# maleiwhat/Our-Tree

Measured on AMD Instinct MI355X. Metric: GB/s AES-128-CTR (whole node), higher is better.
Workload: dtype uint8

## Files before the change

csrc/cpu/bs_selftest.cpp:

```cpp
#include <stdio.h>
#include <stdlib.h>
#include <string.h>

#include "aes.h"
#include "otc_bitslice.h"

using namespace otc_bs;

extern "C" int otc_bitslice_selftest(int verbose)
{
    const uint8_t *SB = aes_sbox();
    int fails = 0;
    for (int batch = 0; batch < 8; ++batch) {
        W x[8] = {0};
        for (int k = 0; k < 32; ++k) {
            int v = batch * 32 + k;
            for (int i = 0; i < 8; ++i) x[i] |= (W)((v >> i) & 1) << k;
        }
        sbox(x[0], x[1], x[2], x[3], x[4], x[5], x[6], x[7]);
        for (int k = 0; k < 32; ++k) {
            int v = batch * 32 + k, o = 0;
            for (int i = 0; i < 8; ++i) o |= (int)((x[i] >> k) & 1) << i;
            if (o != SB[v]) {
                if (verbose) printf("  sbox mismatch at %02x: %02x vs %02x\n", v, o, SB[v]);
                ++fails;
            }
        }
    }
    for (int kv = 0; kv < 256; kv += 37) {
        W k[8], x[8] = {0}, y[8];
        for (int i = 0; i < 8; ++i) k[i] = ((kv >> i) & 1) ? ~0u : 0u;
        for (int slot = 0; slot < 32; ++slot)
            for (int i = 0; i < 8; ++i) x[i] |= (W)(((slot * 7 + kv) >> i) & 1) << slot;
        for (int i = 0; i < 8; ++i) y[i] = x[i] ^ k[i];
        sbox(y[0], y[1], y[2], y[3], y[4], y[5], y[6], y[7]);
        W z[8];
        for (int i = 0; i < 8; ++i) z[i] = x[i];
        sbox_k<false>(x[0], x[1], x[2], x[3], x[4], x[5], x[6], x[7], k[0], k[1], k[2], k[3], k[4], k[5], k[6], k[7]);
        sbox_lut3(z[0], z[1], z[2], z[3], z[4], z[5], z[6], z[7], k[0], k[1], k[2], k[3], k[4], k[5], k[6], k[7]);
        for (int i = 0; i < 8; ++i)
            if (x[i] != y[i] || z[i] != y[i]) {
                if (verbose) printf("  sbox_k/sbox_lut3 mismatch kv=%d bit %d\n", kv, i);
                ++fails;
            }
    }
    for (int t = 0; t < 64; ++t) {
        W a[32], b[32];
        uint64_t z = 0x9E3779B97F4A7C15ull * (uint64_t)(t + 1);
        for (int i = 0; i < 32; ++i) {
            z ^= z << 13; z ^= z >> 7; z ^= z << 17;
            a[i] = b[i] = (W)(z >> 11);
        }
        transpose32(a);
        transpose32_ref(b);
        for (int i = 0; i < 32; ++i)
            if (a[i] != b[i]) {
                if (verbose) printf("  transpose32 mismatch (trial %d, word %d)\n", t, i);
                ++fails;
                break;
            }
    }
    srand(7);
    for (int bits = 128; bits <= 256; bits += 64) {
        unsigned char key[32], pt[32][16], ref[32][16];
        for (int i = 0; i < 32; ++i) key[i] = (unsigned char)rand();
        for (int k = 0; k < 32; ++k)
            for (int i = 0; i < 16; ++i) pt[k][i] = (unsigned char)rand();
        aes_context ctx;
        aes_setkey_enc(&ctx, key, (unsigned)bits);
        for (int k = 0; k < 32; ++k) aes_crypt_ecb(&ctx, AES_ENCRYPT, pt[k], ref[k]);
        uint32_t rk[60];
        aes_export_rk32(&ctx, rk);
        W s[128];
        for (int w = 0; w < 4; ++w) {
            W m[32];
            for (int k = 0; k < 32; ++k) memcpy(&m[k], &pt[k][4 * w], 4);
            transpose32(m);
            for (int q = 0; q < 32; ++q) s[32 * w + q] = m[q];
        }
        W km[128];
        key_masks(rk, km);
        for (int p = 0; p < 128; ++p) s[p] ^= km[p];
        for (int r = 1; r < ctx.nr; ++r) {
            key_masks(rk + 4 * r, km);
            round_full(s, km);
        }
        key_masks(rk + 4 * ctx.nr, km);
        round_last(s, km);
        int bad = 0;
        for (int w = 0; w < 4; ++w) {
            W m[32];
            for (int q = 0; q < 32; ++q) m[q] = s[32 * w + q];
            transpose32(m);
            for (int k = 0; k < 32; ++k) bad += memcmp(&m[k], &ref[k][4 * w], 4) != 0;
        }
        if (verbose) printf("  bitsliced AES-%d (32 blocks): %s\n", bits, bad ? "failed" : "passed");
        fails += bad;

        for (int w = 0; w < 4; ++w) {
            W m[32];
            for (int k = 0; k < 32; ++k) memcpy(&m[k], &pt[k][4 * w], 4);
            transpose32(m);
            for (int q = 0; q < 32; ++q) s[32 * w + q] = m[q];
        }
        auto kf = [&](int r, int p) -> W { return (W)(0u - ((rk[4 * r + (p >> 5)] >> (p & 31)) & 1u)); };
        if (ctx.nr == 10) encrypt_planes<10, false>(s, kf);
        else if (ctx.nr == 12) encrypt_planes<12, false>(s, kf);
        else encrypt_planes<14, false>(s, kf);
        bad = 0;
        for (int w = 0; w < 4; ++w) {
            W m[32];
            for (int q = 0; q < 32; ++q) m[q] = s[32 * w + q];
            transpose32(m);
            for (int k = 0; k < 32; ++k) {
                uint32_t v = m[k] ^ rk[4 * ctx.nr + w];
                bad += memcmp(&v, &ref[k][4 * w], 4) != 0;
            }
        }
        if (verbose) printf("  bitsliced AES-%d kernel schedule: %s\n", bits, bad ? "failed" : "passed");
        fails += bad;

        for (int mixt = 0; mixt < 3; ++mixt) {
            for (int w = 0; w < 4; ++w) {
                W m[32];
                for (int k = 0; k < 32; ++k) memcpy(&m[k], &pt[k][4 * w], 4);
                transpose32(m);
                for (int q = 0; q < 32; ++q) s[32 * w + q] = m[q];
            }
            for (int r = 0; r + 1 < ctx.nr; ++r) {
                auto kr = [&](int p) -> W { return kf(r, p); };
                if (mixt == 2) round_step<2>(s, kr);
                else if (mixt == 1) round_step<1>(s, kr);
                else round_step<0>(s, kr);
            }
            round_final(s, [&](int p) -> W { return kf(ctx.nr - 1, p); });
            bad = 0;
            for (int w = 0; w < 4; ++w) {
                W m[32];
                for (int q = 0; q < 32; ++q) m[q] = s[32 * w + q];
                transpose32(m);
// ... 102 lines not shown
```

csrc/hip/aes_bs.hip:

```cpp
#include <hip/hip_runtime.h>

#include <cstdlib>
#include <cstring>
#include <type_traits>

#include "otc_bitslice.h"
#include "otc_device.h"
#include "otc_kernels.h"

using namespace otc_dev;
using namespace otc_bs;

namespace {

struct BsParams {
    const uint8_t *in;
    uint8_t *out;
    uint64_t nblocks;
    uint32_t tail;
    uint32_t wrap64;
    uint64_t shift;
    Ctr128 cbase;
    const uint32_t *ktab;
    const uint32_t *ctab;
// ... 149 lines not shown
    __device__ __forceinline__ void operator()(int b, W *t) const
    {
        ktab_ptr q = tp;
        asm volatile("" : "+s"(q));
#pragma unroll
        for (int j = 0; j < OTC_SBOX_KEY_TERMS; ++j) t[j] = q[(R * 16 + b) * OTC_BS_KT_STRIDE + j];
    }
};

template <int BASE>
struct GroupTerms {
    ktab_ptr gp;
    __device__ __forceinline__ void operator()(int b, W *t) const
    {
        ktab_ptr q = gp;
        asm volatile("" : "+s"(q));
#pragma unroll
        for (int j = 0; j < OTC_SBOX_KEY_TERMS; ++j) t[j] = q[(BASE + b) * OTC_BS_KT_STRIDE + j];
    }
};

__global__ __launch_bounds__(256) void k_bs_ctr_table(otc_aes_key K, Ctr128 cbase, uint32_t wrap64,
                                                      uint64_t ngroups, uint64_t tasks, uint32_t *gtab,
                                                      uint32_t *e0tab, uint32_t *e1tab)
{
    __shared__ uint32_t sbt[256];
    sbt[threadIdx.x] = sbox_value(threadIdx.x);
    __syncthreads();
    const auto sb = [&](uint32_t v) { return sbt[v & 0xFFu]; };
    const uint64_t i = (uint64_t)blockIdx.x * 256u + threadIdx.x;
    auto rk0b = [&](int b) -> uint32_t { return (K.rk[b >> 2] >> (8 * (b & 3))) & 0xFFu; };
    uint64_t g;
    int kind;
    if (i < ngroups) {
        g = i;
        kind = 0;
    } else if (i < ngroups * 65) {
        g = (i - ngroups) >> 6;
        kind = 1;
    } else if (i < ngroups * 65 + tasks) {
        g = (((cbase.lo >> 11) & 31u) + (i - ngroups * 65)) >> 5;
        kind = 2;
    } else {
        return;
    }
    uint8_t pre[14];
    ctr_group_prefix(cbase.lo, cbase.hi, wrap64 != 0, g, pre);
    uint32_t c8[8];
    if (kind == 0) {
        ctr_group_consts(pre, K.rk, sb, c8, gtab + g * OTC_BS_CTR_GRP_WORDS);
    } else if (kind == 1) {
        ctr_group_consts(pre, K.rk, sb, c8, (uint32_t *)nullptr);
        const uint32_t lane = (uint32_t)(i - ngroups) & 63u;
        ctr_e0_lane(c8, rk0b(15), lane, sb, e0tab + (g * 64 + lane) * 8);
    } else {
        ctr_group_consts(pre, K.rk, sb, c8, (uint32_t *)nullptr);
        const uint64_t t = i - ngroups * 65;
        const uint32_t u5 = (uint32_t)((cbase.lo >> 11) + t) & 31u;
        ctr_e1_task(c8, rk0b(14), u5, sb, e1tab + t * OTC_BS_CTR_E1_WORDS);
    }
}

template <int R, int NR, int MIX, bool DEC = false>
__device__ __forceinline__ void rounds_table(W *s, ktab_ptr tp)
{
    if constexpr (R < NR - 1) {
        round_step_kt<MIX, TableTerms<R>, 2, DEC>(s, TableTerms<R>{tp});
        pin_n(s, 128);
        rounds_table<R + 1, NR, MIX, DEC>(s, tp);
    } else {
        round_final_kt<TableTerms<NR - 1>, DEC>(s, TableTerms<NR - 1>{tp});
    }
}

#ifndef OTC_BS_CBC_D
#define OTC_BS_CBC_D 4
#endif
#ifndef OTC_BS_CFB_D
#define OTC_BS_CFB_D 2
#endif
#ifndef OTC_BS_PRE
#define OTC_BS_PRE 2
#endif
template <int NR, int MODE, int LS, bool CACHE, bool FO, int MIX = 2, int PRE = OTC_BS_PRE, int D = 8>
__device__ __forceinline__ void aes_bs_task(const BsParams &P, const otc_aes_key &K, uint4 *stage,
                                            int64_t claimed = -1)
{
    Task t;
    if (!task_of<MODE>(P, t, claimed)) return;
    const uint32_t lane = t.lane, wave = t.wave;
    const uint64_t shift = (MODE == BS_CTR) ? P.shift : 0;
    const bool full = FO || t.full;
    W s[128];
    auto prefetch = [&]() {
    if (MODE == BS_CTR && LS > 0) {
        const int64_t t0 = (int64_t)t.vbase - (int64_t)shift;
        const uint8_t *ib0 = P.in + t0 * 16 + lane * 16u;
#pragma unroll
        for (int k = 0; k < LS; ++k) {
            const int64_t si = t0 + (int64_t)lane + 64 * k;
            const bool ok = full || (si >= 0 && (uint64_t)si < P.nblocks);
            __builtin_amdgcn_global_load_lds((const void *)(ok ? ib0 + 1024u * k : P.in),
                                             (__attribute__((address_space(3))) void *)&stage[(wave * LS + k) * 64],
                                             16, 0, BS_LDS_AUX);
        }
    }
    };
    if (!(MODE == BS_CTR && CACHE)) prefetch();
    if (MODE == BS_CTR && CACHE) {
        const uint64_t task = t.vbase >> 11;
        const uint64_t g = (((P.cbase.lo >> 11) & 31u) + task) >> 5;
        const uint4 *q0 = (const uint4 *)(P.e0tab + (g * 64u + lane) * 8u);
        const uint4 a = q0[0], b = q0[1];
        const W ew[8] = {a.x, a.y, a.z, a.w, b.x, b.y, b.z, b.w};
        W e0[32];
#pragma unroll
        for (int p = 0; p < 32; ++p) e0[p] = rep_byte(ew[p >> 2], p & 3);
        const ktab_ptr e1p = (ktab_ptr)P.e1tab + task * OTC_BS_CTR_E1_WORDS;
        W e1[32];
#pragma unroll
        for (int p = 0; p < 32; ++p) e1[p] = e1p[p];
        const ktab_ptr gp = (ktab_ptr)P.ctab + g * OTC_BS_CTR_GRP_WORDS;
        ctr_round2_mix(e0, e1, s);
        pin_n(s, 128);
        sched_fence();
        prefetch();
        sched_fence();
        round_step_kt<MIX, GroupTerms<0>, 2>(s, GroupTerms<0>{gp});
        pin_n(s, 128);
        sched_fence();
        rounds_table<3, NR, MIX>(s, (ktab_ptr)P.ktab);
    } else if (MODE == BS_CTR) {
        const uint64_t clo = P.cbase.lo + t.vbase;
        const uint64_t chi = P.cbase.hi + ((!P.wrap64 && clo < P.cbase.lo) ? 1u : 0u);
        uint32_t cw[4] = {(uint32_t)clo, (uint32_t)(clo >> 32), (uint32_t)chi, (uint32_t)(chi >> 32)};
#pragma unroll
        for (int j = 0; j < 4; ++j) asm volatile("" : "+v"(cw[j]));
#pragma unroll
        for (int b = 0; b < 16; ++b) {
#pragma unroll
            for (int i = 0; i < 8; ++i) {
                const int n = 8 * (15 - b) + i;
                W v;
                if (n < 6) {
                    v = lane_mask(lane, n);
                } else if (n < 11) {
                    constexpr W pat[5] = {0xAAAAAAAAu, 0xCCCCCCCCu, 0xF0F0F0F0u, 0xFF00FF00u, 0xFFFF0000u};
                    v = pat[n - 6];
                } else {
                    v = (W)(0u - ((cw[n >> 5] >> (n & 31)) & 1u));
                }
                s[8 * b + i] = v;
            }
        }
#pragma unroll
        for (int q = 0; q < 128; ++q) asm volatile("" : "+v"(s[q]));
    } else {
        ecb_load_planes<MODE>(P, t, s, full);
    }
    constexpr bool DEC = MODE == BS_ECB_DEC || is_cbcd<MODE>;
    if (DEC) {
        dec_premap(s);
        pin_n(s, 128);
    }
    if (!(MODE == BS_CTR && CACHE)) {
        sched_fence();
        rounds_table<0, NR, MIX, DEC>(s, (ktab_ptr)P.ktab);
    }
    pin_n(s, 128);
    sched_fence();

    const int64_t tstart = (int64_t)t.vbase - (int64_t)shift;
    const uint8_t *ib = P.in + tstart * 16;
    uint8_t *ob = P.out + tstart * 16;
    uint32_t lo = lane * 16u;
    asm volatile("" : "+v"(lo));
    auto slot_ok = [&](int k) {
        const int64_t si = tstart + (int64_t)lane + 64 * k;
        return full || (si >= 0 && (uint64_t)si < P.nblocks);
    };
    constexpr bool XIN = MODE == BS_CTR || is_cbcd<MODE> || is_cfbd<MODE>;
    constexpr int XOFF = MODE == BS_CBC_DEC ? -16 : 0;
    uint4 pt[32];
    auto issue = [&](int j) {
        if (XIN && j >= LS && j < 32) {
            if constexpr (MODE == BS_CBC_DEC_SEG) {
                pt[j] = seg_prev<MODE>(P, ib + lo + 1024u * j, (uint64_t)(tstart + lane + 64 * j),
                                       slot_ok(j));
            } else if (MODE == BS_CBC_DEC && j == 0) {
                const bool first = tstart + lane == 0;
                const uint4 v = slot_ok(j) ? *(const uint4 *)(ib + lo + (first ? 0 : XOFF)) : make_uint4(0, 0, 0, 0);
                pt[j] = blend_iv(v, first, P);
            } else {
                pt[j] = slot_ok(j) ? ld_stream(ib + lo + 1024u * j + XOFF) : make_uint4(0, 0, 0, 0);
            }
        }
    };
    constexpr bool REG_XIN = is_cbcd<MODE> || is_cfbd<MODE>;
    constexpr int PRE_ = REG_XIN ? 0 : PRE, D_ = is_cfbd<MODE> ? OTC_BS_CFB_D : REG_XIN ? OTC_BS_CBC_D : D;
#pragma unroll
    for (int j = 0; j < LS + PRE_; ++j) issue(j);
    sched_fence();
#pragma unroll
    for (int w = 0; w < 4; ++w) {
        transpose32(s + 32 * w);
        pin_n(s + 32 * w, 32);
        sched_fence();
    }
    constexpr uint32_t KD = DEC ? 0x05050505u : 0u;
    const uint32_t k0 = K.rk[4 * NR + 0] ^ KD, k1 = K.rk[4 * NR + 1] ^ KD, k2 = K.rk[4 * NR + 2] ^ KD,
                   k3 = K.rk[4 * NR + 3] ^ KD;
    auto ks_xor = [&](int k, uint4 x) {
        uint4 o;
        o.x = x3(x.x, s[k], k0);
        o.y = x3(x.y, s[32 + k], k1);
        o.z = x3(x.z, s[64 + k], k2);
        o.w = x3(x.w, s[96 + k], k3);
        return o;
    };
#pragma unroll
    for (int k = 0; k < 32; ++k) {
        if ((k & 3) == 0) {
            sched_fence();
#pragma unroll
            for (int j = LS + PRE_; j < 32; ++j)
                if ((j - D_ < 0 ? 0 : ((j - D_) & ~3)) == k) issue(j);
        }
        if (slot_ok(k)) {
            const uint4 o = XIN ? ks_xor(k, k < LS ? stage[(wave * LS + k) * 64 + (lo >> 4)] : pt[k])
                                : make_uint4(s[k] ^ k0, s[32 + k] ^ k1, s[64 + k] ^ k2, s[96 + k] ^ k3);
            st_stream(ob + lo + 1024u * k, o);
        }
    }
}

#ifndef OTC_BS_LS
#define OTC_BS_LS 8
#endif
constexpr int BS_LS = OTC_BS_LS;


template <int NR, int MODE, int LS, bool CACHE, bool FO>
__global__ __launch_bounds__(256) __attribute__((amdgpu_waves_per_eu(3, 3))) void k_aes_bs_t3(BsParams P,
                                                                                             otc_aes_key K)
{
    __shared__ uint4 stage[LS > 0 ? BS_WPG * LS * 64 : 1];
    aes_bs_task<NR, MODE, LS, CACHE, FO>(P, K, stage);
}

template <int NR, int MODE>
__global__ __launch_bounds__(256) __attribute__((amdgpu_waves_per_eu(3, 3))) void k_aes_bs_claim(BsParams P,
                                                                                               otc_aes_key K)
{
    strace(3);
    const uint32_t w = blockIdx.x * 4u + __builtin_amdgcn_readfirstlane(threadIdx.x >> 6);
    for (int64_t u = first_unit(P.cl, false, w); u >= 0; u = claim_unit(P.cl, false)) {
        BsParams Q = P;
        auto gin = (__attribute__((address_space(1))) const uint8_t *)P.in;
        auto gout = (__attribute__((address_space(1))) uint8_t *)P.out;
        asm volatile("" : "+s"(gin), "+s"(gout));
        Q.in = (const uint8_t *)gin;
        Q.out = (uint8_t *)gout;
        aes_bs_task<NR, MODE, 0, false, true>(Q, K, nullptr, u);
    }
}

template <int NR, int MODE>
hipError_t launch_nr(const BsParams &P, const otc_aes_key &K, hipStream_t st)
{
    const uint64_t vt = P.nblocks + (MODE == BS_CTR ? P.shift : 0);
    const uint64_t tasks = (vt + 2047) / 2048;
    uint64_t wgs = (tasks + BS_WPG - 1) / BS_WPG;
    if (wgs < 1) wgs = 1;
    if (wgs > 0xFFFFFFFFull) return hipErrorInvalidValue;
    const dim3 g((unsigned)wgs), b(64 * BS_WPG);
    bool cache = MODE == BS_CTR;
    const uint64_t ngroups = cache ? (((P.cbase.lo >> 11) & 31u) + tasks + 31) >> 5 : 0;
    const size_t ctab_words =
        cache ? ngroups * (OTC_BS_CTR_GRP_WORDS + OTC_BS_CTR_E0_WORDS) + tasks * OTC_BS_CTR_E1_WORDS : 0;
    const size_t kt_words = (size_t)NR * 16 * OTC_BS_KT_STRIDE;
    uint32_t *tab = nullptr;
    hipError_t e = hipErrorOutOfMemory;
    if (cache) {
        e = alloc_fault() ? hipErrorOutOfMemory : hipMallocAsync((void **)&tab, (kt_words + ctab_words) * 4, st);
        if (e != hipSuccess) {
            (void)hipGetLastError();
            cache = false;
        }
    }
    if (!cache) e = alloc_fault() ? hipErrorOutOfMemory : hipMallocAsync((void **)&tab, kt_words * 4, st);
    if (e != hipSuccess) return e;
    hipLaunchKernelGGL(k_bs_key_table<MODE == BS_ECB_DEC || is_cbcd<MODE>>, dim3(1), dim3(256), 0, st, K, tab);
    BsParams Q = P;
    Q.ktab = tab;
    Q.tasks = tasks;
    constexpr int LS = MODE == BS_CTR ? BS_LS : 0;
    if constexpr (MODE != BS_CTR) {
        (void)g;
        if (!P.cl.ctr) {
            (void)hipFreeAsync(tab, st);
            return hipErrorInvalidValue;
        }
        hipLaunchKernelGGL((k_aes_bs_claim<NR, MODE>),
                           dim3(P.cl.wgs ? P.cl.wgs : (unsigned)otc_dev::device_cus()), dim3(256), 0, st, Q, K);
    } else {
        const bool edge = P.shift != 0 || vt % 2048 != 0;
        auto run = [&](auto cachec) {
            constexpr bool C = decltype(cachec)::value;
            Q.part = BS_FULL_ONLY;
            hipLaunchKernelGGL((k_aes_bs_t3<NR, MODE, LS, C, true>), g, b, 0, st, Q, K);
            if (edge) {
                Q.part = BS_EDGE_ONLY;
                hipLaunchKernelGGL((k_aes_bs_t3<NR, MODE, LS, C, false>), dim3((2 + BS_WPG - 1) / BS_WPG), b, 0, st,
                                   Q, K);
// ... 93 lines not shown
```

csrc/include/otc.h:

```cpp
#ifndef OTC_H
#define OTC_H

#include <stddef.h>
#include <stdint.h>

#ifdef __cplusplus
extern "C" {
#endif

#define OTC_OK 0
#define OTC_ERR_ARG -1
#define OTC_ERR_HIP -2
#define OTC_ERR_RCCL -3
#define OTC_ERR_UNSUPPORTED -4
#define OTC_ERR_NOMEM -5

const char *otc_last_error(void);

#define OTC_DIR_ENCRYPT 1
#define OTC_DIR_DECRYPT 0

typedef struct {
    uint32_t rk[60];
    int32_t nr;
// ... 156 lines not shown
int otc_device_clock_khz(int dev);
int otc_set_device(int dev);
int otc_device_sync(void);
void *otc_stream_create(void);
void otc_stream_destroy(void *stream);
int otc_stream_join(void *a, void *b);

typedef struct otc_engine otc_engine;

otc_engine *otc_engine_create(int device, size_t chunk_bytes, int depth);
#define OTC_ENGINE_DEFAULT 0
#define OTC_ENGINE_POOLED_QUEUES 1
otc_engine *otc_engine_create_ex(int device, size_t chunk_bytes, int depth, int flags);
void otc_engine_destroy(otc_engine *e);

#define OTC_MODE_ECB 0
#define OTC_MODE_CTR 1
#define OTC_MODE_CBC_DEC 2
#define OTC_MODE_XOR 3

typedef struct {
    double total_ms;
    double kernel_ms;
    double h2d_ms, d2h_ms;
    double host_stage_ms;
    size_t bytes;
    int chunks;
    int numa_node;
} otc_stream_stats;

int otc_engine_run(otc_engine *e, int mode, const void *host_in, void *host_out, size_t nbytes,
                   const otc_aes_key *k, const uint8_t iv_or_ctr[16], uint64_t block_offset,
                   int impl, otc_stream_stats *stats);

int otc_device_numa_node(int dev);
int otc_engine_numa_node(const otc_engine *e);
const void *otc_engine_staging(const otc_engine *e, int slot);

#define OTC_PTR_HOST 0
#define OTC_PTR_PINNED 1
#define OTC_PTR_DEVICE 2
int otc_ptr_kind(const void *p);

int otc_host_register(void *p, size_t nbytes);
int otc_host_unregister(void *p);
void *otc_host_alloc_pinned(size_t nbytes);
void otc_host_free_pinned(void *p);

typedef struct {
    double total_ms;
    double gbps;
    int ngpus;
    int strategy;
    int numa_nodes_used;
} otc_multi_stats;

int otc_multi_run(int ngpus, int strategy, int mode, const void *host_in, void *host_out,
                  size_t nbytes, const otc_aes_key *k, const uint8_t iv_or_ctr[16], int impl,
                  size_t chunk_bytes, otc_multi_stats *stats);

typedef struct {
    uint64_t round_off;
    uint64_t round_bytes;
    uint64_t pad_bytes;
    uint64_t off, bytes;
    uint64_t blk0;
    int64_t halo;
} otc_rccl_piece;
uint64_t otc_rccl_nrounds(uint64_t nbytes, int ngpus, uint64_t piece);
int otc_rccl_plan_piece(uint64_t nbytes, int ngpus, uint64_t piece, uint64_t r, int g, otc_rccl_piece *out);
uint64_t otc_rccl_halo_start(uint64_t nbytes, uint64_t piece, uint64_t i);

void otc_multi_release(void);
void otc_release_resources(void);

void otc_fault_inject_alloc(long after);
long otc_fault_inject_pending(void);

int otc_multi_ctr_resident(int ngpus, void *const *dev_bufs, size_t shard_bytes,
                           const otc_aes_key *k, const uint8_t ctr0[16], int impl,
                           double *elapsed_ms);

int otc_bitslice_selftest(int verbose);
const char *otc_build_info(void);
int otc_runtime_info(char *buf, size_t n);

#ifdef __cplusplus
}
#endif

#endif
```

csrc/include/otc_bitslice.h:

```cpp
#ifndef OTC_BITSLICE_H
#define OTC_BITSLICE_H

#include <stdint.h>

#if defined(__HIPCC__) || defined(__HIP__)
#define OTC_HD __host__ __device__ __forceinline__
#else
#define OTC_HD inline
#endif



namespace otc_bs {

typedef uint32_t W;

OTC_HD void sbox(W &x0, W &x1, W &x2, W &x3, W &x4, W &x5, W &x6, W &x7)
{
    const W U0 = x7, U1 = x6, U2 = x5, U3 = x4, U4 = x3, U5 = x2, U6 = x1, U7 = x0;
    const W T1 = U0 ^ U3, T2 = U0 ^ U5, T3 = U0 ^ U6, T4 = U3 ^ U5, T5 = U4 ^ U6;
    const W T6 = T1 ^ T5, T7 = U1 ^ U2, T8 = U7 ^ T6, T9 = U7 ^ T7, T10 = T6 ^ T7;
    const W T11 = U1 ^ U5, T12 = U2 ^ U5, T13 = T3 ^ T4, T14 = T6 ^ T11, T15 = T5 ^ T11;
    const W T16 = T5 ^ T12, T17 = T9 ^ T16, T18 = U3 ^ U7, T19 = T7 ^ T18, T20 = T1 ^ T19;
    const W T21 = U6 ^ U7, T22 = T7 ^ T21, T23 = T2 ^ T22, T24 = T2 ^ T10, T25 = T20 ^ T17;
// ... 578 lines not shown
}

OTC_HD void key_masks(const uint32_t *rk4, W *k)
{
#pragma unroll
    for (int b = 0; b < 16; ++b) {
        uint32_t byte = (rk4[b >> 2] >> (8 * (b & 3))) & 0xffu;
#pragma unroll
        for (int i = 0; i < 8; ++i) k[8 * b + i] = ((byte >> i) & 1u) ? ~0u : 0u;
    }
}

struct ArrayKey {
    const W *k;
    OTC_HD W operator()(int p) const { return k[p]; }
};

OTC_HD void round_full(W *s, const W *k)
{
    W t[128];
    sub_bytes(s);
    shift_rows(s, t);
    mix_columns_ark(t, s, ArrayKey{k});
}

OTC_HD void round_last(W *s, const W *k)
{
    W t[128];
    sub_bytes(s);
    shift_rows(s, t);
#pragma unroll
    for (int p = 0; p < 128; ++p) s[p] = t[p] ^ k[p];
}

OTC_HD W perm_b(W hi, W lo, uint32_t sel)
{
#if defined(__HIP_DEVICE_COMPILE__)
    return __builtin_amdgcn_perm(hi, lo, sel);
#else
    W r = 0;
    for (int i = 0; i < 4; ++i) {
        const uint32_t s = (sel >> (8 * i)) & 0xFFu;
        const W byte = s < 4 ? (lo >> (8 * s)) & 0xFFu : (hi >> (8 * (s - 4))) & 0xFFu;
        r |= byte << (8 * i);
    }
    return r;
#endif
}

OTC_HD W bsel(W m, W x, W y) { return (x & m) | (y & ~m); }

template <int J>
OTC_HD void transpose_bits(W *m, W mk)
{
#pragma unroll
    for (int k = 0; k < 32; ++k) {
        if (k & J) continue;
        const W a = m[k], b = m[k | J];
        m[k] = bsel(mk << J, b << J, a);
        m[k | J] = bsel(mk, a >> J, b);
    }
}

OTC_HD void transpose32(W *m)
{
#pragma unroll
    for (int k = 0; k < 16; ++k) {
        const W a = m[k], b = m[k | 16];
        m[k] = perm_b(b, a, 0x05040100u);
        m[k | 16] = perm_b(b, a, 0x07060302u);
    }
#pragma unroll
    for (int k = 0; k < 32; ++k) {
        if (k & 8) continue;
        const W a = m[k], b = m[k | 8];
        m[k] = perm_b(b, a, 0x06020400u);
        m[k | 8] = perm_b(b, a, 0x07030501u);
    }
    transpose_bits<4>(m, 0x0F0F0F0Fu);
    transpose_bits<2>(m, 0x33333333u);
    transpose_bits<1>(m, 0x55555555u);
}

inline void transpose32_ref(W *m)
{
    W t[32] = {0};
    for (int r = 0; r < 32; ++r)
        for (int c = 0; c < 32; ++c) t[c] |= ((m[r] >> c) & 1u) << r;
    for (int i = 0; i < 32; ++i) m[i] = t[i];
}

}

#endif
```

our_tree_amd/_native.py:

```python
from __future__ import annotations

import atexit
import ctypes
import os
import threading

_HERE = os.path.dirname(os.path.abspath(__file__))
LIB_DIR = os.path.join(_HERE, "lib")
GPU_LIB_PATH = os.environ.get("OTC_LIB") or os.path.join(LIB_DIR, "libotc.so")
CPU_LIB_PATH = os.path.join(LIB_DIR, "libotc_cpu.so")

_lock = threading.Lock()
_gpu_lib = None
_cpu_lib = None

c_u8p = ctypes.POINTER(ctypes.c_uint8)
c_vp = ctypes.c_void_p
c_sz = ctypes.c_size_t
c_u64 = ctypes.c_uint64
c_int = ctypes.c_int


class OtcAesKey(ctypes.Structure):

# ... 49 lines not shown

    _fields_ = [("nonce_counter", ctypes.c_uint8 * 16), ("stream_block", ctypes.c_uint8 * 16),
                ("nc_off", ctypes.c_size_t)]


class StreamStats(ctypes.Structure):
    _fields_ = [
        ("total_ms", ctypes.c_double),
        ("kernel_ms", ctypes.c_double),
        ("h2d_ms", ctypes.c_double),
        ("d2h_ms", ctypes.c_double),
        ("host_stage_ms", ctypes.c_double),
        ("bytes", ctypes.c_size_t),
        ("chunks", ctypes.c_int),
        ("numa_node", ctypes.c_int),
    ]


class RcclPiece(ctypes.Structure):
    _fields_ = [
        ("round_off", ctypes.c_uint64),
        ("round_bytes", ctypes.c_uint64),
        ("pad_bytes", ctypes.c_uint64),
        ("off", ctypes.c_uint64),
        ("bytes", ctypes.c_uint64),
        ("blk0", ctypes.c_uint64),
        ("halo", ctypes.c_int64),
    ]


class MultiStats(ctypes.Structure):
    _fields_ = [
        ("total_ms", ctypes.c_double),
        ("gbps", ctypes.c_double),
        ("ngpus", ctypes.c_int),
        ("strategy", ctypes.c_int),
        ("numa_nodes_used", ctypes.c_int),
    ]


def _declare_cpu(lib):
    P = ctypes.POINTER
    sig = {
        "aes_setkey_enc": (c_int, [P(AesContext), c_u8p, ctypes.c_uint]),
        "aes_setkey_dec": (c_int, [P(AesContext), c_u8p, ctypes.c_uint]),
        "aes_crypt_ecb": (c_int, [P(AesContext), c_int, c_u8p, c_u8p]),
        "aes_crypt_cbc": (c_int, [P(AesContext), c_int, c_sz, c_u8p, c_u8p, c_u8p]),
        "aes_crypt_cfb128": (c_int, [P(AesContext), c_int, c_sz, P(c_int), c_u8p, c_u8p, c_u8p]),
        "aes_crypt_ctr": (c_int, [P(AesContext), c_int, P(c_int), c_u8p, c_u8p, c_u8p, c_u8p]),
        "aes_self_test": (c_int, [c_int]),
        "aes_export_rk32": (c_int, [P(AesContext), P(ctypes.c_uint32)]),
        "aes_ctr_bulk": (c_int, [P(AesContext), c_u8p, c_u8p, c_u8p, c_sz, c_int]),
        "aes_ecb_bulk": (c_int, [P(AesContext), c_int, c_u8p, c_u8p, c_sz, c_int]),
        "aes_ctr128_add": (None, [c_u8p, c_u64]),
        "aes_xts_setkey_enc": (c_int, [P(AesXtsContext), c_u8p, ctypes.c_uint]),
        "aes_xts_setkey_dec": (c_int, [P(AesXtsContext), c_u8p, ctypes.c_uint]),
        "aes_crypt_xts": (c_int, [P(AesXtsContext), c_int, c_sz, c_u8p, c_u8p, c_u8p]),
        "aes_crypt_xts_units": (c_int, [P(AesXtsContext), c_int, c_sz, c_sz, c_u8p, c_u8p, c_u8p]),
        "aes_gcm_setkey": (c_int, [P(AesGcmContext), c_u8p, ctypes.c_uint]),
        "aes_gcm_set_h": (None, [P(AesGcmContext), c_u8p]),
        "aes_gf128_mul": (None, [c_u8p, c_u8p, c_u8p]),
        "aes_ghash": (None, [P(AesGcmContext), c_u8p, c_u8p, c_sz]),
        "aes_gcm_j0": (None, [P(AesGcmContext), c_u8p, c_sz, c_u8p]),
        "aes_crypt_ctr32": (c_int, [P(AesGcmContext), c_sz, c_u8p, c_u8p, c_u8p]),
        "aes_crypt_gcm": (c_int, [P(AesGcmContext), c_int, c_sz, c_u8p, c_sz, c_u8p, c_sz, c_u8p, c_u8p, c_u8p]),
        "aes_gcm_auth_decrypt": (c_int, [P(AesGcmContext), c_sz, c_u8p, c_sz, c_u8p, c_sz, c_u8p, c_sz, c_u8p, c_u8p]),
        "arc4_setup": (None, [P(Arc4Context), c_u8p, ctypes.c_uint]),
        "arc4_prep": (c_int, [P(Arc4Context), c_sz, c_u8p]),
        "arc4_crypt": (c_int, [c_sz, c_u8p, c_u8p, c_u8p]),
        "arc4_crypt_mt": (c_int, [c_sz, c_u8p, c_u8p, c_u8p, c_int]),
        "arc4_self_test": (c_int, [c_int]),
        "rc4_init": (None, [P(Rc4State), ctypes.c_char_p, c_int]),
        "rc4_crypt": (None, [P(Rc4State), ctypes.c_char_p, ctypes.c_char_p, c_int]),
        "CheckAESSupport": (c_int, []),
        "AES_128_Key_Expansion": (None, [c_u8p, c_u8p]),
        "AES_192_Key_Expansion": (None, [c_u8p, c_u8p]),
        "AES_256_Key_Expansion": (None, [c_u8p, c_u8p]),
        "AES_Key_Expansion_Dec": (None, [c_u8p, c_u8p, c_int]),
        "AES_ECB_encrypt": (None, [c_u8p, c_u8p, ctypes.c_ulong, c_u8p, c_int]),
        "AES_ECB_decrypt": (None, [c_u8p, c_u8p, ctypes.c_ulong, c_u8p, c_int]),
        "AES_CTR_encrypt": (None, [c_u8p, c_u8p, c_u8p, c_u8p, ctypes.c_ulong, c_u8p, c_int]),
        "AES_CTR_encrypt_at": (None, [c_u8p, c_u8p, c_u8p, c_u8p, ctypes.c_ulong, c_u8p, c_int, ctypes.c_ulonglong]),
        "otc_bitslice_selftest": (c_int, [c_int]),
        "otc_rccl_nrounds": (c_u64, [c_u64, c_int, c_u64]),
        "otc_rccl_plan_piece": (c_int, [c_u64, c_int, c_u64, c_u64, c_int, P(RcclPiece)]),
        "otc_rccl_halo_start": (c_u64, [c_u64, c_u64, c_u64]),
        "AES_CBC_encrypt": (None, [c_u8p, c_u8p, c_u8p, ctypes.c_ulong, c_u8p, c_int]),
        "AES_CFB128_encrypt": (None, [c_u8p, c_u8p, c_u8p, ctypes.c_ulong, c_u8p, c_int]),
        "aes_monte_carlo": (c_int, [c_int, c_int, c_u8p]),
        "aes_monte_carlo_expected": (ctypes.c_char_p, [c_int, c_int]),
        "otc_parse_cpulist": (c_int, [ctypes.c_char_p, c_u8p, c_int]),
        "otc_numa_node_of_pci": (c_int, [ctypes.c_char_p, ctypes.c_char_p]),
        "otc_numa_node_cpus": (c_int, [ctypes.c_char_p, c_int, c_u8p, c_int]),
        "otc_numa_num_nodes": (c_int, [ctypes.c_char_p]),
        "otc_numa_bind_thread": (c_int, [c_int]),
        "otc_numa_alloc": (c_vp, [c_sz, c_int]),
        "otc_numa_free": (None, [c_vp, c_sz]),
        "otc_numa_node_of_addr": (c_int, [c_vp]),
    }
    for name, (res, args) in sig.items():
        fn = getattr(lib, name)
        fn.restype = res
        fn.argtypes = args


def _declare_gpu(lib):
    _declare_cpu(lib)
    P = ctypes.POINTER
    K = P(OtcAesKey)
    sig = {
        "otc_last_error": (ctypes.c_char_p, []),
        "otc_pick_impl": (c_int, [c_int, c_int, c_int, c_u64]),
        "otc_last_impl": (c_int, []),
        "otc_xts_key_init": (c_int, [P(OtcXtsKey), c_u8p, c_int, c_int]),
        "otc_aes_xts": (c_int, [c_vp, c_vp, c_sz, c_sz, P(OtcXtsKey), c_u8p, c_vp]),
        "otc_gcm_key_init": (c_int, [P(OtcGcmKey), c_u8p, c_int]),
        "otc_aes_ctr32": (c_int, [c_vp, c_vp, c_sz, K, c_u8p, c_int, c_vp]),
        "otc_ghash": (c_int, [c_vp, c_sz, c_u8p, c_u8p, c_vp, c_vp]),
        "otc_aes_gcm": (c_int, [c_vp, c_vp, c_sz, P(OtcGcmKey), c_int, c_u8p, c_sz, c_u8p, c_sz, c_vp, c_int, c_vp]),
        "otc_ghash_spans": (c_int, [P(c_u64), c_int]),
        "otc_gcm_batch_spans": (c_int, [P(c_u64), c_int]),
        "otc_gcm_batch_table_bytes": (c_sz, []),
        "otc_gcm_batch_ws_bytes": (c_sz, [c_sz]),
        "otc_gcm_batch_tables": (c_int, [P(OtcGcmKey), c_vp, c_vp]),
        "otc_gcm_batch_plan": (ctypes.c_int64, [c_vp, c_sz, c_int, c_vp, c_vp, c_vp]),
        "otc_gcm_batch_lanes": (c_int, [c_vp, c_sz]),
        "otc_ghash_batch": (c_int, [c_vp, c_sz, c_vp, c_vp, c_int, c_vp]),
        "otc_aes_gcm_batch": (c_int, [c_vp, c_vp, c_vp, c_vp, c_u64, c_int, c_sz, P(OtcGcmKey), c_vp, c_vp, c_int,
                                      c_vp, c_vp, c_vp, c_int, c_vp, c_vp, c_int, c_vp]),
        "otc_split_stats": (None, [c_int]),
        "otc_split_fallback_reason": (ctypes.c_char_p, []),
        "otc_split_last_units": (c_int, [ctypes.POINTER(c_u64), ctypes.POINTER(c_u64), ctypes.POINTER(c_u64)]),
        "otc_aes_key_init": (c_int, [K, c_u8p, c_int, c_int]),
        "otc_aes_ecb": (c_int, [c_vp, c_vp, c_sz, K, c_int, c_vp]),
        "otc_aes_ctr": (c_int, [c_vp, c_vp, c_sz, K, c_u8p, c_u64, c_int, c_vp]),
        "otc_aes_ctr_rfc3686": (c_int, [c_vp, c_vp, c_sz, K, c_u8p, c_u8p, c_u64, c_int, c_vp]),
        "otc_aes_ctr_ctx_init": (c_int, [P(OtcCtrCtx), c_u8p]),
        "otc_aes_ctr_stream": (c_int, [P(OtcCtrCtx), K, c_sz, c_vp, c_vp, c_int, c_vp]),
        "otc_aes_cbc_decrypt": (c_int, [c_vp, c_vp, c_sz, K, c_u8p, c_vp]),
        "otc_aes_cbc_decrypt_impl": (c_int, [c_vp, c_vp, c_sz, K, c_u8p, c_int, c_vp]),
        "otc_stream_create": (c_vp, []),
        "otc_dev_malloc": (c_vp, [c_sz]),
        "otc_dev_free": (None, [c_vp]),
        "otc_memcpy": (c_int, [c_vp, c_vp, c_sz, c_int]),
        "otc_stream_destroy": (None, [c_vp]),
        "otc_stream_join": (c_int, [c_vp, c_vp]),
        "otc_aes_cbc_encrypt_segments": (c_int, [c_vp, c_vp, c_sz, c_sz, K, c_u8p, c_vp]),
        "otc_aes_cbc_encrypt_segments_impl": (c_int, [c_vp, c_vp, c_sz, c_sz, K, c_u8p, c_int, c_vp]),
        "otc_aes_cfb128_encrypt_segments_impl": (c_int, [c_vp, c_vp, c_sz, c_sz, K, c_u8p, c_int, c_vp]),
        "otc_aes_cbc_decrypt_segments": (c_int, [c_vp, c_vp, c_sz, c_sz, K, c_u8p, c_vp]),
        "otc_aes_cfb128_decrypt": (c_int, [c_vp, c_vp, c_sz, K, c_u8p, c_vp]),
        "otc_aes_cfb128_decrypt_impl": (c_int, [c_vp, c_vp, c_sz, K, c_u8p, c_int, c_vp]),
        "otc_aes_cfb128_encrypt_segments": (c_int, [c_vp, c_vp, c_sz, c_sz, K, c_u8p, c_vp]),
        "otc_aes_cfb128_decrypt_segments": (c_int, [c_vp, c_vp, c_sz, c_sz, K, c_u8p, c_vp]),
        "otc_aes_cfb128_decrypt_segments_impl": (c_int, [c_vp, c_vp, c_sz, c_sz, K, c_u8p, c_int, c_vp]),
        "otc_aes_cbc_decrypt_segments_impl": (c_int, [c_vp, c_vp, c_sz, c_sz, K, c_u8p, c_int, c_vp]),
        "otc_aes_ctr_batch": (c_int, [c_vp, c_vp, c_vp, c_vp, c_u64, c_int, c_int, c_vp]),
        "otc_xor": (c_int, [c_vp, c_vp, c_vp, c_sz, c_vp]),
        "otc_rc4_multi": (c_int, [c_vp, c_int, c_sz, c_sz, c_sz, c_vp, c_vp, c_vp]),
        "otc_rc4_crypt_batch": (c_int, [c_vp, c_sz, c_sz, c_vp, c_vp, c_vp]),
        "otc_fill_random": (c_int, [c_vp, c_sz, c_u64, c_vp]),
        "otc_checksum": (c_int, [c_vp, c_sz, c_vp, c_vp]),
        "otc_clock_probe": (c_int, [c_vp, ctypes.c_double, ctypes.c_double, c_vp]),
        "otc_AES_ECB_encrypt": (c_int, [c_vp, c_vp, ctypes.c_ulong, c_u8p, c_int, c_vp]),
        "otc_AES_ECB_decrypt": (c_int, [c_vp, c_vp, ctypes.c_ulong, c_u8p, c_int, c_vp]),
        "otc_AES_CTR_encrypt": (c_int, [c_vp, c_vp, c_u8p, c_u8p, ctypes.c_ulong, c_u8p, c_int, c_vp]),
# ... 109 lines not shown
```

Measured before the change: 1703.

## Interleave bitslice output transpose with per-quad stores and loads in CTR

In CTR mode the bitsliced state is now un-transposed depth-first. A byte-level shuffle runs first, then the nibble and bit swap stages are finished one quad of output words at a time. Each finished quad is stored immediately, and further input loads are issued under a look-ahead cap. The goal is to overlap the output transpose with global stores and loads, and to lower peak register pressure compared with transposing all 128 words before any store. Host-side model and test helpers are added to check the new transpose order and issue schedule. The risk is a worse instruction schedule or extra register spills if the compiler does not honour the fences.

```diff
diff --git a/csrc/cpu/bs_selftest.cpp b/csrc/cpu/bs_selftest.cpp
--- a/csrc/cpu/bs_selftest.cpp
+++ b/csrc/cpu/bs_selftest.cpp
@@ -2,10 +2,77 @@
 #include <stdlib.h>
 #include <string.h>
 
+#include <utility>
+
 #include "aes.h"
 #include "otc_bitslice.h"
 
 using namespace otc_bs;
+
+
+template <int... G, int... Q>
+static void dfs_step(W *m, int step, std::integer_sequence<int, G...>, std::integer_sequence<int, Q...>)
+{
+    ((step == G ? transpose32_nib8<G>(m) : (void)0), ...);
+    ((step == 8 + Q ? transpose32_quad<Q>(m) : (void)0), ...);
+    ((step == 16 + G ? transpose32_group8<G>(m) : (void)0), ...);
+}
+
+extern "C" int otc_bs_dfs_transpose(uint32_t *m, const int *steps, int nsteps)
+{
+    for (int i = 0; i < nsteps; ++i) {
+        const int s = steps[i];
+        if (!((s >= 0 && s < 4) || (s >= 8 && s < 16) || (s >= 16 && s < 20))) return -1;
+    }
+    transpose32_bytes(m);
+    for (int i = 0; i < nsteps; ++i)
+        dfs_step(m, steps[i], std::make_integer_sequence<int, 4>{}, std::make_integer_sequence<int, 8>{});
+    return 0;
+}
+
+extern "C" int otc_bs_ctr_out_model(const uint32_t *planes, const uint32_t *rk, const uint32_t *pt, uint32_t *out,
+                                    int dfs, int ls, int first, int cap, int *order)
+{
+    W s[128];
+    for (int p = 0; p < 128; ++p) s[p] = planes[p];
+    int issued[32], emitted[32], nemit = 0, err = 0;
+    uint32_t reg[32][4];
+    for (int k = 0; k < 32; ++k) {
+        issued[k] = k < first;
+        emitted[k] = 0;
+        for (int w = 0; w < 4; ++w) reg[k][w] = issued[k] ? pt[4 * k + w] : 0xDEADBEEFu;
+        if (order) order[k] = -1;
+    }
+    auto emit = [&](int k) {
+        if (!issued[k]) err = err ? err : 1;
+        if (emitted[k]++) err = err ? err : 2;
+        for (int w = 0; w < 4; ++w) out[4 * k + w] = x3(reg[k][w], s[32 * w + k], rk[w]);
+        ++nemit;
+    };
+    auto issue = [&](int j) {
+        if (j < first || issued[j]++) err = err ? err : 2;
+        for (int w = 0; w < 4; ++w) reg[j][w] = pt[4 * j + w];
+        if (order) order[j] = nemit;
+    };
+    if (!dfs) {
+        for (int w = 0; w < 4; ++w) transpose32(s + 32 * w);
+        for (int j = first; j < 32; ++j) issue(j);
+        for (int k = 0; k < 32; ++k) emit(k);
+    } else if (ls == 8 && first == 10 && cap == 36) {
+        ctr_out_dfs<8, 10, 36>(s, emit, issue);
+    } else if (ls == 8 && first == 10 && cap == 34) {
+        ctr_out_dfs<8, 10, 34>(s, emit, issue);
+    } else if (ls == 12 && first == 14 && cap == 36) {
+        ctr_out_dfs<12, 14, 36>(s, emit, issue);
+    } else if (ls == 0 && first == 4 && cap == 40) {
+        ctr_out_dfs<0, 4, 40>(s, emit, issue);
+    } else {
+        return -1;
+    }
+    for (int k = 0; k < 32; ++k)
+        if (!issued[k] || emitted[k] != 1) err = err ? err : 2;
+    return err;
+}
 
 extern "C" int otc_bitslice_selftest(int verbose)
 {
@@ -51,11 +118,21 @@
             z ^= z << 13; z ^= z >> 7; z ^= z << 17;
             a[i] = b[i] = (W)(z >> 11);
         }
+        W c[32];
+        for (int i = 0; i < 32; ++i) c[i] = a[i];
         transpose32(a);
         transpose32_ref(b);
         for (int i = 0; i < 32; ++i)
             if (a[i] != b[i]) {
                 if (verbose) printf("  transpose32 mismatch (trial %d, word %d)\n", t, i);
+                ++fails;
+                break;
+            }
+        const int rev[4] = {19, 18, 17, 16};
+        otc_bs_dfs_transpose(c, rev, 4);
+        for (int i = 0; i < 32; ++i)
+            if (c[i] != b[i]) {
+                if (verbose) printf("  depth-first transpose mismatch (trial %d, word %d)\n", t, i);
                 ++fails;
                 break;
             }
diff --git a/csrc/hip/aes_bs.hip b/csrc/hip/aes_bs.hip
--- a/csrc/hip/aes_bs.hip
+++ b/csrc/hip/aes_bs.hip
@@ -255,6 +255,14 @@
 #ifndef OTC_BS_PRE
 #define OTC_BS_PRE 2
 #endif
+#ifndef OTC_BS_OUT_DFS
+#define OTC_BS_OUT_DFS 1
+#endif
+#ifndef OTC_BS_DFS_CAP
+#define OTC_BS_DFS_CAP 36
+#endif
+constexpr bool BS_OUT_DFS = OTC_BS_OUT_DFS != 0;
+constexpr int BS_DFS_CAP = OTC_BS_DFS_CAP;
 template <int NR, int MODE, int LS, bool CACHE, bool FO, int MIX = 2, int PRE = OTC_BS_PRE, int D = 8>
 __device__ __forceinline__ void aes_bs_task(const BsParams &P, const otc_aes_key &K, uint4 *stage,
                                             int64_t claimed = -1)
@@ -374,12 +382,6 @@
 #pragma unroll
     for (int j = 0; j < LS + PRE_; ++j) issue(j);
     sched_fence();
-#pragma unroll
-    for (int w = 0; w < 4; ++w) {
-        transpose32(s + 32 * w);
-        pin_n(s + 32 * w, 32);
-        sched_fence();
-    }
     constexpr uint32_t KD = DEC ? 0x05050505u : 0u;
     const uint32_t k0 = K.rk[4 * NR + 0] ^ KD, k1 = K.rk[4 * NR + 1] ^ KD, k2 = K.rk[4 * NR + 2] ^ KD,
                    k3 = K.rk[4 * NR + 3] ^ KD;
@@ -391,18 +393,31 @@
         o.w = x3(x.w, s[96 + k], k3);
         return o;
     };
-#pragma unroll
-    for (int k = 0; k < 32; ++k) {
-        if ((k & 3) == 0) {
-            sched_fence();
-#pragma unroll
-            for (int j = LS + PRE_; j < 32; ++j)
-                if ((j - D_ < 0 ? 0 : ((j - D_) & ~3)) == k) issue(j);
-        }
+    auto emit = [&](int k) {
         if (slot_ok(k)) {
             const uint4 o = XIN ? ks_xor(k, k < LS ? stage[(wave * LS + k) * 64 + (lo >> 4)] : pt[k])
                                 : make_uint4(s[k] ^ k0, s[32 + k] ^ k1, s[64 + k] ^ k2, s[96 + k] ^ k3);
             st_stream(ob + lo + 1024u * k, o);
+        }
+    };
+    if constexpr (BS_OUT_DFS && MODE == BS_CTR && LS + PRE_ >= 4) {
+        ctr_out_dfs<LS, LS + PRE_, BS_DFS_CAP>(s, emit, issue);
+    } else {
+#pragma unroll
+        for (int w = 0; w < 4; ++w) {
+            transpose32(s + 32 * w);
+            pin_n(s + 32 * w, 32);
+            sched_fence();
+        }
+#pragma unroll
+        for (int k = 0; k < 32; ++k) {
+            if ((k & 3) == 0) {
+                sched_fence();
+#pragma unroll
+                for (int j = LS + PRE_; j < 32; ++j)
+                    if ((j - D_ < 0 ? 0 : ((j - D_) & ~3)) == k) issue(j);
+            }
+            emit(k);
         }
     }
 }
diff --git a/csrc/include/otc.h b/csrc/include/otc.h
--- a/csrc/include/otc.h
+++ b/csrc/include/otc.h
@@ -262,6 +262,9 @@
                            double *elapsed_ms);
 
 int otc_bitslice_selftest(int verbose);
+int otc_bs_dfs_transpose(uint32_t *m, const int *steps, int nsteps);
+int otc_bs_ctr_out_model(const uint32_t *planes, const uint32_t *rk, const uint32_t *pt, uint32_t *out, int dfs,
+                         int ls, int first, int cap, int *order);
 const char *otc_build_info(void);
 int otc_runtime_info(char *buf, size_t n);
 
diff --git a/csrc/include/otc_bitslice.h b/csrc/include/otc_bitslice.h
--- a/csrc/include/otc_bitslice.h
+++ b/csrc/include/otc_bitslice.h
@@ -684,6 +684,110 @@
     transpose_bits<1>(m, 0x55555555u);
 }
 
+
+OTC_HD void transpose32_bytes(W *m)
+{
+#pragma unroll
+    for (int k = 0; k < 16; ++k) {
+        const W a = m[k], b = m[k | 16];
+        m[k] = perm_b(b, a, 0x05040100u);
+        m[k | 16] = perm_b(b, a, 0x07060302u);
+    }
+#pragma unroll
+    for (int k = 0; k < 32; ++k) {
+        if (k & 8) continue;
+        const W a = m[k], b = m[k | 8];
+        m[k] = perm_b(b, a, 0x06020400u);
+        m[k | 8] = perm_b(b, a, 0x07030501u);
+    }
+}
+
+template <int J, int LO, int N>
+OTC_HD void transpose_bits_in(W *m, W mk)
+{
+    static_assert(N % (2 * J) == 0 && LO % N == 0 && LO + N <= 32, "whole swap pairs only");
+#pragma unroll
+    for (int k = LO; k < LO + N; ++k) {
+        if (k & J) continue;
+        const W a = m[k], b = m[k | J];
+        m[k] = bsel(mk << J, b << J, a);
+        m[k | J] = bsel(mk, a >> J, b);
+    }
+}
+
+template <int G>
+OTC_HD void transpose32_nib8(W *m)
+{
+    transpose_bits_in<4, 8 * G, 8>(m, 0x0F0F0F0Fu);
+}
+
+template <int Q>
+OTC_HD void transpose32_quad(W *m)
+{
+    transpose_bits_in<2, 4 * Q, 4>(m, 0x33333333u);
+    transpose_bits_in<1, 4 * Q, 4>(m, 0x55555555u);
+}
+
+template <int G>
+OTC_HD void transpose32_group8(W *m)
+{
+    transpose32_nib8<G>(m);
+    transpose32_quad<2 * G>(m);
+    transpose32_quad<2 * G + 1>(m);
+}
+
+OTC_HD void pin4x4(W *a, W *b, W *c, W *d)
+{
+#if defined(__HIP_DEVICE_COMPILE__)
+    asm volatile(""
+                 : "+v"(a[0]), "+v"(a[1]), "+v"(a[2]), "+v"(a[3]), "+v"(b[0]), "+v"(b[1]), "+v"(b[2]), "+v"(b[3]),
+                   "+v"(c[0]), "+v"(c[1]), "+v"(c[2]), "+v"(c[3]), "+v"(d[0]), "+v"(d[1]), "+v"(d[2]), "+v"(d[3]));
+#else
+    (void)a, (void)b, (void)c, (void)d;
+#endif
+}
+
+constexpr int ctr_out_dfs_limit(int q, int ls, int first, int cap)
+{
+    const int done = 4 * (q + 1);
+    const int lim = cap - 32 + done + (done > ls ? done : ls);
+    return q < 0 || lim < first ? first : lim > 32 ? 32 : lim;
+}
+
+template <int Q, int LS, int FIRST, int CAP, class Emit, class Issue>
+OTC_HD void ctr_out_dfs_quad(W *s, Emit &emit, Issue &issue)
+{
+    constexpr int LIM = ctr_out_dfs_limit(Q, LS, FIRST, CAP);
+    static_assert(Q == 7 || LIM >= 4 * (Q + 2), "look-ahead too short: raise CAP");
+#pragma unroll
+    for (int w = 0; w < 4; ++w) {
+        if (Q % 2 == 0) transpose32_nib8<Q / 2>(s + 32 * w);
+        transpose32_quad<Q>(s + 32 * w);
+    }
+    pin4x4(s + 4 * Q, s + 32 + 4 * Q, s + 64 + 4 * Q, s + 96 + 4 * Q);
+    sched_fence();
+#pragma unroll
+    for (int i = 0; i < 4; ++i) emit(4 * Q + i);
+    sched_fence();
+#pragma unroll
+    for (int j = ctr_out_dfs_limit(Q - 1, LS, FIRST, CAP); j < LIM; ++j) issue(j);
+    sched_fence();
+    if constexpr (Q < 7) ctr_out_dfs_quad<Q + 1, LS, FIRST, CAP>(s, emit, issue);
+}
+
+template <int LS, int FIRST, int CAP, class Emit, class Issue>
+OTC_HD void ctr_out_dfs(W *s, Emit emit, Issue issue)
+{
+    static_assert(FIRST >= 4 && FIRST >= LS && FIRST <= 32, "quad 0's slots are ready before the phase");
+#pragma unroll
+    for (int w = 0; w < 4; ++w) {
+        transpose32_bytes(s + 32 * w);
+        pin_n(s + 32 * w, 32);
+        sched_fence();
+    }
+    ctr_out_dfs_quad<0, LS, FIRST, CAP>(s, emit, issue);
+}
+
 inline void transpose32_ref(W *m)
 {
     W t[32] = {0};
diff --git a/our_tree_amd/_native.py b/our_tree_amd/_native.py
--- a/our_tree_amd/_native.py
+++ b/our_tree_amd/_native.py
@@ -155,6 +155,9 @@
         "AES_CTR_encrypt": (None, [c_u8p, c_u8p, c_u8p, c_u8p, ctypes.c_ulong, c_u8p, c_int]),
         "AES_CTR_encrypt_at": (None, [c_u8p, c_u8p, c_u8p, c_u8p, ctypes.c_ulong, c_u8p, c_int, ctypes.c_ulonglong]),
         "otc_bitslice_selftest": (c_int, [c_int]),
+        "otc_bs_dfs_transpose": (c_int, [P(ctypes.c_uint32), P(c_int), c_int]),
+        "otc_bs_ctr_out_model": (c_int, [P(ctypes.c_uint32), P(ctypes.c_uint32), P(ctypes.c_uint32),
+                                         P(ctypes.c_uint32), c_int, c_int, c_int, c_int, P(c_int)]),
         "otc_rccl_nrounds": (c_u64, [c_u64, c_int, c_u64]),
         "otc_rccl_plan_piece": (c_int, [c_u64, c_int, c_u64, c_u64, c_int, P(RcclPiece)]),
         "otc_rccl_halo_start": (c_u64, [c_u64, c_u64, c_u64]),
```

Result: faster. 1725, median of 6 (+1.3%).
